# zzhang1987/Factor-Graph-Neural-Network

Measured on AMD Instinct MI355X. Metric: VF+FV messages/sec on 96.3.963 LDPC graph, higher is better.
Workload: dtype bf16

## Files before the change

factor-graph-neural-network_amd/csrc/bnact.hip:

```cpp
#include "fgnn_common.h"
#include "fgnn_device.h"
#include "fgnn_gridfold.h"
#include <stdlib.h>

#define BN_THREADS 256
#define BN_GRID 512
#define BN_MAXPART 1024
#define BN_APPLY_GRID 4096

struct BnParams {
    const void* x;
    const void* gy;
    void* out;
    float* ws;
    const float* a;
    const float* b;
    const float* gamma;
    const float* beta;
    const float* ref;
    const void* addend;
    const void* addend2;
    const void* addend3;
    int aperiod[3];
    int64_t R;
// ... 118 lines not shown
        for (int q = pg * 8; q < pg * 8 + 8; ++q) { a += red0[q * BN_FC + cc]; b += red1[q * BN_FC + cc]; }
    __syncthreads();
    if (pg < 8) { red0[threadIdx.x] = a; red1[threadIdx.x] = b; }
    __syncthreads();
    s0 = 0.0; s1 = 0.0;
    if (pg == 0)
        for (int q = 0; q < 8; ++q) { s0 += red0[q * BN_FC + cc]; s1 += red1[q * BN_FC + cc]; }
}

__global__ __launch_bounds__(256) void bn_stats_final_kernel(const float* ws, int nwg, int C, const fgnn_bn_final fin) {
    if (fin.num_batches_tracked && blockIdx.x == 0 && threadIdx.x == 0) *fin.num_batches_tracked += 1;
    const int c = blockIdx.x * BN_FC + (threadIdx.x & (BN_FC - 1)), pg = threadIdx.x / BN_FC;
    double s0, s1;
    bn_fold(ws, nwg, C, c, pg, c < C, s0, s1);
    if (pg != 0 || c >= C) return;
    const double n = (double)fin.count;
    const double m0 = s0 / n;
    double var = s1 / n - m0 * m0;
    if (var < 0.0) var = 0.0;
    const float mu = (float)(m0 + (fin.shift_k ? (double)fin.shift_k[c] : 0.0));
    const float is = (float)(1.0 / sqrt(var + (double)fin.eps));
    fin.mean[c] = mu;
    fin.invstd[c] = is;
    const float g = fin.gamma ? fin.gamma[c] : 1.f, b = fin.beta ? fin.beta[c] : 0.f;
    fin.scale[c] = g * is;
    fin.shift[c] = b - mu * g * is;
    if (fin.running_mean) {
        const double np = (double)(fin.population > 0 ? fin.population : fin.count);
        const double unbiased = np > 1.0 ? var * np / (np - 1.0) : var;
        fin.running_mean[c] = (1.f - fin.momentum) * fin.running_mean[c] + fin.momentum * mu;
        fin.running_var[c] = (1.f - fin.momentum) * fin.running_var[c] + fin.momentum * (float)unbiased;
    }
}

__global__ __launch_bounds__(256) void bn_bwd_final_kernel(const float* ws, int nwg, int C, float* dsum,
                                                           float* gweight, float* gbias) {
    const int c = blockIdx.x * BN_FC + (threadIdx.x & (BN_FC - 1)), pg = threadIdx.x / BN_FC;
    double s0, s1;
    bn_fold(ws, nwg, C, c, pg, c < C, s0, s1);
    if (pg != 0 || c >= C) return;
    dsum[c] = (float)s0;
    dsum[C + c] = (float)s1;
    if (gbias) gbias[c] += (float)s0;
    if (gweight) gweight[c] += (float)s1;
}

template <typename T, int MODE>
__global__ __launch_bounds__(BN_THREADS) void bn_apply_kernel(const BnParams p) {
    constexpr int EPC = Chunk<T>::EPC;
    const int tid = threadIdx.x;
    const int cpr = 1 << p.cshift;
    const int cg = tid & (cpr - 1), rg = tid >> p.cshift;
    const int rstep = BN_THREADS >> p.cshift;
    const int c0 = cg * EPC;
    const T* xg = static_cast<const T*>(p.x);
    const T* gg = static_cast<const T*>(p.gy);
    T* og = static_cast<T*>(p.out);
    float ka[EPC], kb[EPC], kc[EPC], kd[EPC], ke[EPC], kf[EPC];
#pragma unroll
// ... 77 lines not shown
}

extern "C" int64_t fgnn_bn_workspace_bytes(int64_t R, int C) { return (int64_t)BN_MAXPART * 2 * C * 4 + 2 * C * 4; }

static int g_inkernel_finalisers = -1;
int fgnn_separate_finalisers(void) {
    if (g_inkernel_finalisers < 0) g_inkernel_finalisers = 0;
    return !g_inkernel_finalisers;
}
extern "C" int fgnn_set_inkernel_finalisers(int on) {
    const int was = !fgnn_separate_finalisers();
    g_inkernel_finalisers = on ? 1 : 0;
    return was;
}

static int bn_check_final(const char* who, const fgnn_bn_final* fin) {
    if (!fin || !fin->mean || !fin->invstd || !fin->scale || !fin->shift) FGNN_FAIL(FGNN_EINVAL, "%s: null pointer in fgnn_bn_final", who);
    if (fin->count < 1 || (fin->population != 0 && fin->population < fin->count)) FGNN_FAIL(FGNN_EINVAL, "%s: bad row counts in fgnn_bn_final", who);
    if ((fin->running_mean == nullptr) != (fin->running_var == nullptr)) FGNN_FAIL(FGNN_EINVAL, "%s: running_mean and running_var go together", who);
    return FGNN_OK;
}

int fgnn_bn_finalize_launch(const float* partials, int npartials, int C, const fgnn_bn_final* fin, hipStream_t st) {
    hipLaunchKernelGGL(bn_stats_final_kernel, dim3((C + BN_FC - 1) / BN_FC), dim3(256), 0, st, partials, npartials, C, *fin);
    return hipGetLastError() == hipSuccess ? 0 : -1;
}

extern "C" int fgnn_bn_stats(const void* x, int64_t R, int C, int dtype, const fgnn_bn_final* fin, void* workspace,
                             int64_t workspace_bytes, void* fold_scratch, fgnn_stream_t stream) {
    BnParams p = {};
    int grid, rc;
    if (!x || !workspace) FGNN_FAIL(FGNN_EINVAL, "bn_stats: null pointer");
    if ((rc = bn_check_final("bn_stats", fin))) return rc;
    if (fin->count != R) FGNN_FAIL(FGNN_EINVAL, "bn_stats: fin->count must be R");
    if (bn_plan(R, C, dtype, &p, &grid)) FGNN_FAIL(FGNN_EUNSUPPORTED, "bn: C=%d not a supported channel count", C);
    if (workspace_bytes < fgnn_bn_workspace_bytes(R, C)) FGNN_FAIL(FGNN_EINVAL, "bn: workspace too small");
    float* ws = (float*)workspace;
    hipStream_t st = (hipStream_t)stream;
    const float* ref = dtype == FGNN_F32 ? (const float*)x : nullptr;
    p.x = x; p.ws = ws; p.ref = ref;
    p.fin = *fin;
    if (ref) {
        if (fin->shift_k) FGNN_FAIL(FGNN_EINVAL, "bn_stats: shift_k is for partials produced elsewhere");
        p.fin.shift_k = ref;
    }
    const bool inkernel = fold_scratch && 2 * C <= FGNN_FOLD_MAXJ && !fgnn_separate_finalisers();
    p.fold = fgnn_fold_make(ws, inkernel ? fold_scratch : nullptr, grid, C);
    if (dtype == FGNN_F32) hipLaunchKernelGGL((bn_reduce_kernel<float, 0>), dim3(grid), dim3(BN_THREADS), 0, st, p);
    else hipLaunchKernelGGL((bn_reduce_kernel<bf16_t, 0>), dim3(grid), dim3(BN_THREADS), 0, st, p);
    if (!inkernel) hipLaunchKernelGGL(bn_stats_final_kernel, dim3((C + BN_FC - 1) / BN_FC), dim3(256), 0, st, ws, grid, C, p.fin);
    hipError_t e = hipGetLastError();
    if (e != hipSuccess) FGNN_FAIL(FGNN_ELAUNCH, "bn_stats launch: %s", hipGetErrorString(e));
    return FGNN_OK;
}

extern "C" int fgnn_bn_finalize(const float* partials, int npartials, int C, const fgnn_bn_final* fin, fgnn_stream_t stream) {
    int rc;
    if (!partials) FGNN_FAIL(FGNN_EINVAL, "bn_finalize: null pointer");
    if ((rc = bn_check_final("bn_finalize", fin))) return rc;
    if (npartials < 1 || npartials > BN_MAXPART || C < 1) FGNN_FAIL(FGNN_EINVAL, "bn_finalize: bad sizes");
    if (fgnn_bn_finalize_launch(partials, npartials, C, fin, (hipStream_t)stream))
        FGNN_FAIL(FGNN_ELAUNCH, "bn_finalize launch: %s", hipGetErrorString(hipGetLastError()));
    return FGNN_OK;
}

extern "C" int fgnn_bn_apply(const void* x, void* y, int64_t R, int C, int dtype, const float* scale,
                             const float* shift, float slope, const void* addend, const void* addend2,
                             const void* addend3, const int32_t* addend_period, fgnn_stream_t stream) {
    BnParams p = {};
    int grid;
    if (!x || !y || !scale || !shift) FGNN_FAIL(FGNN_EINVAL, "bn_apply: null pointer");
    if (bn_plan(R, C, dtype, &p, &grid, bn_apply_grid())) FGNN_FAIL(FGNN_EUNSUPPORTED, "bn: C=%d not a supported channel count", C);
    p.x = x; p.out = y; p.a = scale; p.b = shift; p.slope = slope; p.addend = addend; p.addend2 = addend2; p.addend3 = addend3;
    for (int a = 0; a < 3; ++a) {
// ... 53 lines not shown
    pa.fold.tickets = nullptr;
    (void)bn_plan(R, C, dtype, &pa, &agrid, bn_apply_grid());
    if (dtype == FGNN_F32) hipLaunchKernelGGL((bn_apply_kernel<float, 1>), dim3(agrid), dim3(BN_THREADS), 0, st, pa);
    else hipLaunchKernelGGL((bn_apply_kernel<bf16_t, 1>), dim3(agrid), dim3(BN_THREADS), 0, st, pa);
    hipError_t e = hipGetLastError();
    if (e != hipSuccess) FGNN_FAIL(FGNN_ELAUNCH, "bn_backward launch: %s", hipGetErrorString(e));
    return FGNN_OK;
}

__global__ __launch_bounds__(256) void bn_bwd_final_raw_kernel(const float* ws, int nwg, int C, const float* mean,
                                                               const float* invstd, float* dsum, float* gweight, float* gbias) {
    const int c = blockIdx.x * BN_FC + (threadIdx.x & (BN_FC - 1)), pg = threadIdx.x / BN_FC;
    double s0, s1;
    bn_fold(ws, nwg, C, c, pg, c < C, s0, s1);
    if (pg != 0 || c >= C) return;
    const double dg = (double)invstd[c] * (s1 - (double)mean[c] * s0);
    dsum[c] = (float)s0;
    dsum[C + c] = (float)dg;
    if (gbias) gbias[c] += (float)s0;
    if (gweight) gweight[c] += (float)dg;
}

int fgnn_bn_bwd_final_raw_launch(const float* partials, int npartials, int C, const float* mean, const float* invstd, float* dsum,
                                 float* gweight, float* gbias, hipStream_t st) {
    hipLaunchKernelGGL(bn_bwd_final_raw_kernel, dim3((C + BN_FC - 1) / BN_FC), dim3(256), 0, st, partials, npartials, C, mean,
                       invstd, dsum, gweight, gbias);
    return hipGetLastError() == hipSuccess ? 0 : -1;
}

extern "C" int fgnn_bn_backward_apply(const void* x, const void* gy, void* gx, int64_t R, int C, int dtype,
                                      const float* mean, const float* invstd, const float* gamma, const float* beta,
                                      float slope, const float* dsum, fgnn_stream_t stream) {
    BnParams p = {};
    int grid;
    if (!x || !gy || !gx || !mean || !invstd || !gamma || !beta || !dsum)
// ... 12 lines not shown
```

factor-graph-neural-network_amd/csrc/fgnn_common.h:

```cpp
#pragma once
#include <hip/hip_runtime.h>
#include <stdint.h>
#include <stdio.h>
#include <stdarg.h>

#include "fgnn_hip.h"

typedef float f32x4 __attribute__((ext_vector_type(4)));

#define FGNN_THREADS 256
#define FGNN_WAVES 4

struct bf16_t { uint16_t v; };

__device__ __forceinline__ float fgnn_ld(const float* p) { return *p; }
__device__ __forceinline__ float fgnn_ld(const bf16_t* p) {
    return __uint_as_float(((uint32_t)p->v) << 16);
}
__device__ __forceinline__ void fgnn_st(float* p, float v) { *p = v; }
__device__ __forceinline__ void fgnn_st(bf16_t* p, float v) {
    const __bf16 h = (__bf16)v;
    p->v = __builtin_bit_cast(uint16_t, h);
}

// ... 18 lines not shown

#ifdef FGNN_ENABLE_PROF
long long* fgnn_prof_begin();
void fgnn_prof_print(const long long* prof, const char* tag, int first, int rows, int cols, int stride);
#else
static inline long long* fgnn_prof_begin() { return nullptr; }
static inline void fgnn_prof_print(const long long*, const char*, int, int, int, int) {}
#endif

static inline int fgnn_round_up(int v, int m) { return (v + m - 1) / m * m; }

void fgnn_launch_slab_reduce(const float* ws, int nslab, int64_t slab_len, int64_t nw, float* gW, float* gbias, hipStream_t st);
void fgnn_launch_slab_reduce_ld(const float* ws, int nslab, int64_t slab_len, int64_t nw, int ncols, int ld, float* gW,
                                float* gbias, hipStream_t st);
bool fgnn_fold_push(const float* ws, int nslab, int64_t slab_len, int64_t nw, float* gW, float* gb, int kind, int a, int b, int c, int d);
int fgnn_bn_finalize_launch(const float* partials, int npartials, int C, const fgnn_bn_final* fin, hipStream_t st);
int fgnn_bn_bwd_final_raw_launch(const float* partials, int npartials, int C, const float* mean, const float* invstd, float* dsum,
                                 float* gweight, float* gbias, hipStream_t st);
int fgnn_bn_backward_sums_bf16(const void* x, const void* gy, int64_t R, int C, const float* mean, const float* invstd,
                               const float* gamma, const float* beta, float slope, float* gweight, float* gbias,
                               void* workspace, void* fold_scratch, hipStream_t st, const float** dsum_out);
```

factor-graph-neural-network_amd/csrc/fgnn_gridfold.h:

```cpp
#pragma once
#include "fgnn_common.h"

#define FGNN_FOLD_GROUP 16
#define FGNN_FOLD_MAXGROUPS 64
#define FGNN_FOLD_MAXJ 512
#define FGNN_FOLD_TICKET_BYTES 512
#define FGNN_FOLD_BYTES (FGNN_FOLD_TICKET_BYTES + FGNN_FOLD_MAXGROUPS * FGNN_FOLD_MAXJ * 8)

struct FgnnFold {
    float* part;
    double* part2;
    unsigned* tickets;
    int rows;
    int row_stride, half_stride, ch;
};

static inline FgnnFold fgnn_fold_make(float* part, void* scratch, int rows, int ch, int row_stride = 0, int half_stride = 0) {
    FgnnFold f;
    f.part = part;
    f.tickets = (unsigned*)scratch;
    f.part2 = scratch ? (double*)((char*)scratch + FGNN_FOLD_TICKET_BYTES) : nullptr;
    f.rows = rows; f.ch = ch;
    f.row_stride = row_stride ? row_stride : 2 * ch;
    f.half_stride = half_stride ? half_stride : ch;
// ... 48 lines not shown
    if (!fgnn_fold_flag) return false;
    for (int j = tid; j < J; j += T) {
        double a = 0.0;
#pragma unroll 8
        for (int q = 0; q < ng; ++q) a += __hip_atomic_load(f.part2 + (int64_t)q * J + j, __ATOMIC_RELAXED, __HIP_MEMORY_SCOPE_AGENT);
        sums[j] = a;
    }
    if (tid == 0) __hip_atomic_store(f.tickets, 0u, __ATOMIC_RELAXED, __HIP_MEMORY_SCOPE_AGENT);
    __syncthreads();
    return true;
}


__device__ __forceinline__ void fgnn_bn_final_apply(const fgnn_bn_final& fin, int ch, const double* sums) {
    if (fin.num_batches_tracked && threadIdx.x == 0) *fin.num_batches_tracked += 1;
    for (int c = threadIdx.x; c < ch; c += blockDim.x) {
        const double n = (double)fin.count;
        const double m0 = sums[c] / n;
        double var = sums[ch + c] / n - m0 * m0;
        if (var < 0.0) var = 0.0;
        const float mu = (float)(m0 + (fin.shift_k ? (double)fin.shift_k[c] : 0.0));
        const float is = (float)(1.0 / sqrt(var + (double)fin.eps));
        fin.mean[c] = mu;
        fin.invstd[c] = is;
        const float g = fin.gamma ? fin.gamma[c] : 1.f, b = fin.beta ? fin.beta[c] : 0.f;
        fin.scale[c] = g * is;
        fin.shift[c] = b - mu * g * is;
        if (fin.running_mean) {
            const double np = (double)(fin.population > 0 ? fin.population : fin.count);
            const double unbiased = np > 1.0 ? var * np / (np - 1.0) : var;
            fin.running_mean[c] = (1.f - fin.momentum) * fin.running_mean[c] + fin.momentum * mu;
            fin.running_var[c] = (1.f - fin.momentum) * fin.running_var[c] + fin.momentum * (float)unbiased;
        }
    }
}

__device__ __forceinline__ void fgnn_bn_bwd_final_apply(int ch, const double* sums, const float* mean, const float* invstd,
                                                        float* dsum, float* gweight, float* gbias) {
    for (int c = threadIdx.x; c < ch; c += blockDim.x) {
        const double s0 = sums[c];
        const double s1 = mean ? (double)invstd[c] * (sums[ch + c] - (double)mean[c] * s0) : sums[ch + c];
        dsum[c] = (float)s0;
        dsum[ch + c] = (float)s1;
        if (gbias) gbias[c] += (float)s0;
        if (gweight) gweight[c] += (float)s1;
    }
}
#endif
```

factor-graph-neural-network_amd/fgnn_amd/_hip.py:

```python
import ctypes
import os
import re

import torch

_HERE = os.path.dirname(os.path.abspath(__file__))
LIB_PATH = os.environ.get('FGNN_HIP_LIB') or os.path.join(_HERE, 'libfgnn_hip.so')
HEADER_PATH = os.path.normpath(os.path.join(_HERE, '..', '..', 'include', 'fgnn_hip.h'))


class FgnnHipError(RuntimeError):
    pass


class MPConvDesc(ctypes.Structure):
    _fields_ = [(n, ctypes.c_int32) for n in
                ('B', 'nin', 'nou', 'net', 'N', 'M', 'k', 'ext', 'agg', 'dtype', 'relu', 'reserved')] + \
               [(n, ctypes.c_int64) for n in
                ('x_sb', 'x_sc', 'x_sn', 'idx_sb', 'idx_sm', 'idx_sk',
                 'et_sb', 'et_se', 'et_sm', 'et_sk', 'y_sb', 'y_sc', 'y_sm')]


class BnFinal(ctypes.Structure):
    _fields_ = [(n, ctypes.c_void_p) for n in ('gamma', 'beta', 'running_mean', 'running_var', 'num_batches_tracked',
# ... 77 lines not shown
            raise FgnnHipError('include/fgnn_hip.h: FGNN_%s = `%s` is not an integer expression' % (name, value.strip()))
        out[name] = int(eval(value, {'__builtins__': {}}))
    return out


def _header():
    if not os.path.exists(HEADER_PATH):
        raise FgnnHipError('the C-ABI header was not found at %s — the binding is derived from it and has no built-in '
                           'copy of the interface' % HEADER_PATH)
    with open(HEADER_PATH) as f:
        return f.read()


SIGNATURES, _K = (parse(_header()) for parse in (signatures, constants))
EXPORTS = tuple(SIGNATURES)
EXT_NONE, EXT_NEIGHBOR, EXT_DIFF = _K['EXT_NONE'], _K['EXT_NEIGHBOR'], _K['EXT_DIFF']
DESC_GETYPE_REDUCED = _K['DESC_GETYPE_REDUCED']
DESC_IDENTITY_LIST = _K['DESC_IDENTITY_LIST']
AGG_MAX, AGG_LSE, AGG_MEAN = _K['AGG_MAX'], _K['AGG_LSE'], _K['AGG_MEAN']
F32, BF16 = _K['F32'], _K['BF16']
DEC_F32, DEC_BF16, DEC_U8 = _K['DEC_F32'], _K['DEC_BF16'], _K['DEC_U8']
LABEL_I64, LABEL_U8 = _K['LABEL_I64'], _K['LABEL_U8']
PGM_DEC_F32, PGM_DEC_BF16, PGM_DEC_I64 = _K['PGM_DEC_F32'], _K['PGM_DEC_BF16'], _K['PGM_DEC_I64']
ABI_VERSION = _K['ABI_VERSION']
EUNSUPPORTED = _K['EUNSUPPORTED']
FOLD_SCRATCH_BYTES = _K['FOLD_SCRATCH_BYTES']

AGG_CODES = {'max': AGG_MAX, 'softmax': AGG_LSE, 'mean': AGG_MEAN}


# ... 91 lines not shown
```

factor-graph-neural-network_amd/fgnn_amd/mpnn/blocks.py:

```python
import ctypes

import torch

from .. import _hip, ops
from . import pointwise
from .message_op import _EXT_CODE, base_mp_nn, mp_conv_type, mp_conv_v2
from .pointwise import (BatchNormAct2d, BnHandoff, NodeInstanceNorm, PointwiseConv2d, _InstNormAct, _RowLinear, as_addends, node_sum,
                        refresh_in_place)
from .pointwise import state_epoch as pointwise_state_epoch


def _conv_norm_act(cin, cout, norm, act, bias=True):
    layers = [PointwiseConv2d(cin, cout, 1, bias=bias)]
    if norm is not None:
        layers.append(norm)
    layers.append(act)
    return torch.nn.Sequential(*layers)


FUSE_EVAL_BLOCKS = True


class iid_mapping(torch.nn.Module):
    def __init__(self, nin, nout, bias=True):
# ... 83 lines not shown
TAIL_WGRAD_MOMENTS = True
FUSE_TRAIN_TAIL = True


FUSE_TRAIN_HEAD = True


_HEAD_WIDTHS = (64, 128)


class _BlockHead(torch.autograd.Function):

    @staticmethod
    def forward(ctx, rows, weight, bias, bn_w, bn_b, handoff, slope, box=None):
        ctx.box = box
        z1 = pointwise.hip_linear(rows, weight, bias, bn=handoff)
        if z1 is None:
            raise _hip.FgnnHipError('fused block head: the 1x1 map is outside csrc/linear_fwd_b16.hip (checked by the caller)')
        R = rows.shape[0]
        stats = handoff.batch_stats(z1)
        a1 = torch.empty_like(z1)
        ops.timed('bn_apply (forward)', 2 * z1.numel() * 2, lambda: _hip.call(
            'fgnn_bn_apply', z1, a1, R, 64, _hip.BF16, stats[2], stats[3], slope, None, None, None, None))
        ctx.save_for_backward(rows, z1, stats, weight, bn_w, bn_b)
        ctx.slope = slope
        ctx.params = (weight, bias, bn_w, bn_b)
        return a1

    @staticmethod
    def backward(ctx, ga1):
        ops.backward_node_begins()
        L = _hip.lib()
        rows, z1, stats, weight, bn_w, bn_b = ctx.saved_tensors
        pW, pbias, pw, pb = ctx.params
        R, cin = rows.shape
        dev = rows.device
        ga1 = ga1.contiguous()
        if ga1.dtype != z1.dtype:
# ... 292 lines not shown
                return y
        M = ops.single_source_fanout(node_feature, nn_idx, etype) if (staged and not self.with_residual and addend is None
                                                                     and node_feature.shape[0] > 1) else 0
        if M:
            B, C = node_feature.shape[:2]
            one = node_feature.reshape(B, 1, 1, C).permute(0, 3, 1, 2)
            y1 = self._forward_staged(one, nn_idx[:, :1, :], etype[:, :, :1, :], None, M)
            return ops.broadcast_nodes(y1, M)
        return self._forward_staged(node_feature, nn_idx, etype, addend, 1)

    def _forward_staged(self, node_feature, nn_idx, etype, addend, mult):
        fuse = self.training
        h = self._fused_train_head(node_feature)
        if h is None:
            handoff = BnHandoff.of(self.conv1[1]) if fuse else None
            h = self.conv1[1](self.conv1[0](node_feature, bn=handoff), handoff=handoff)
        y = self._fused_train_tail(h, nn_idx, etype, addend, mult)
        if y is not None:
            return y + node_feature if self.with_residual else y
        h = self.mp_conv(h, nn_idx, etype, population_mult=mult)
        handoff = BnHandoff.of(self.conv2[1]) if (fuse and mult == 1) else None
        h = self.conv2[0](h, bn=handoff)
        if callable(addend):
            addend = addend()
        h = self.conv2[1](h, addend=addend, population_mult=mult, handoff=handoff)
        return h + node_feature if self.with_residual else h

    def _fused_train_head(self, x):
        conv, bn = self.conv1[0], self.conv1[1]
        handoff = BnHandoff.of(bn) if isinstance(bn, BatchNormAct2d) else None
        if not (FUSE_TRAIN_HEAD and self.training and torch.is_grad_enabled() and x.is_cuda and isinstance(conv, PointwiseConv2d)
# ... 75 lines not shown
```

factor-graph-neural-network_amd/fgnn_amd/mpnn/pointwise.py:

```python
import ctypes
import dataclasses
import weakref

import torch

from .. import _hip, ops


_CAST_CACHE = {}
_CAST_EPOCH = 0
_FLAT_MIRRORS = []


def invalidate_casts():
    global _CAST_EPOCH
    _CAST_EPOCH += 1


_STATE_EPOCH = 0


def note_state_change():
    global _STATE_EPOCH
    _STATE_EPOCH += 1
# ... 47 lines not shown
        v = _from_flat_mirror(t, dtype)
        if v is not None:
            return v
    key = id(t)
    hit = _CAST_CACHE.get(key)
    if hit is not None and hit[0]() is t and hit[3].dtype == dtype and hit[3].device == t.device and hit[3].shape == t.shape:
        if hit[1] != t._version or hit[2] != _CAST_EPOCH:
            hit[3].copy_(t.detach())
            hit[1], hit[2] = t._version, _CAST_EPOCH
        return hit[3]
    out = t.detach().to(dtype)
    _CAST_CACHE[key] = [weakref.ref(t, lambda _, key=key: _CAST_CACHE.pop(key, None)), t._version, _CAST_EPOCH, out]
    return out


@dataclasses.dataclass(eq=False)
class BnHandoff:
    gamma: torch.Tensor
    beta: torch.Tensor
    running_mean: torch.Tensor
    running_var: torch.Tensor
    num_batches_tracked: torch.Tensor
    momentum: float
    eps: float
    rows: torch.Tensor = dataclasses.field(default=None, init=False)
    stats: torch.Tensor = dataclasses.field(default=None, init=False)

    @classmethod
    def of(cls, bn):
        if bn is None or not bn.training or not bn.track_running_stats or not bn.affine or bn.momentum is None:
# ... 12 lines not shown
        note_state_change()
        self.rows, self.stats = rows, stats

    def stats_for(self, rows):
        if self.stats is not None and self.rows.data_ptr() == rows.data_ptr() and self.rows.shape == rows.shape:
            return self.stats
        return None

    def batch_stats(self, rows, population=0):
        stats = self.stats_for(rows)
        if stats is not None:
            return stats
        L = _hip.lib()
        R, C = rows.shape
        stats, fin = self.final(C, rows.device, R, population, running=self.stats is None)
        ws = ops._workspace(rows.device, int(L.fgnn_bn_workspace_bytes(R, C)))
        fold = ops._fold_scratch(rows.device)
        ops.timed('bn_stats (reduce + finalise)', rows.numel() * rows.element_size(), lambda: _hip.call(
            'fgnn_bn_stats', rows, R, C, _hip.dtype_code(rows), fin, ws, ws.numel() * 4, fold))
        note_state_change()
        return stats


def hip_linear(rows, weight, bias, bn=None, transposed=False):
    if not (rows.is_cuda and rows.dtype == torch.bfloat16 and weight.dtype == torch.float32 and rows.is_contiguous()):
        return None
    R, cin = rows.shape
    cout = weight.shape[1] if transposed else weight.shape[0]
    if cin * cout > (16384 if bn is not None else 8192):
        return None
# ... 251 lines not shown
            periods.append(1)
    return ts, periods


def period_array(periods):
    periods = (list(periods) + [1, 1, 1])[:3]
    return None if all(q == 1 for q in periods) else (ctypes.c_int32 * 3)(*periods)


class _BatchNormAct(torch.autograd.Function):

    @staticmethod
    def forward(ctx, rows, weight, bias, handoff, slope, addend=None, addend2=None, addend3=None, periods=(1, 1, 1), population=0):
        R, C = rows.shape
        dt = _hip.dtype_code(rows)
        stats = handoff.batch_stats(rows, population)
        y = torch.empty_like(rows)
        ctx.has_addend = tuple(a is not None for a in (addend, addend2, addend3))
        ctx.periods = tuple(periods)
        ops.timed('bn_apply (forward)', (2 + sum(ctx.has_addend)) * rows.numel() * rows.element_size(),
                  lambda: _hip.call('fgnn_bn_apply', rows, y, R, C, dt, stats[2], stats[3], slope, addend, addend2, addend3,
                                    period_array(periods)))
        ctx.save_for_backward(rows, weight, bias, stats)
        ctx.slope = slope
        ctx.params = (weight, bias)
        return y

    @staticmethod
    def backward(ctx, gy):
        ops.backward_node_begins()
        rows, weight, bias, stats = ctx.saved_tensors
        L = _hip.lib()
        R, C = rows.shape
        gy = gy.contiguous()
        if gy.dtype != rows.dtype:
            gy = gy.to(rows.dtype)
        gx = torch.empty_like(rows)
        grads = ops.param_grads(rows.device)
        gw, gb = grads.acc('gamma', ctx.params[0], (C,)), grads.acc('beta', ctx.params[1], (C,))
        ws = ops._workspace(rows.device, int(L.fgnn_bn_workspace_bytes(R, C)))
        fold = ops._fold_scratch(rows.device)
        ops.timed('bn_backward (reduce + finalise + apply)', 5 * rows.numel() * rows.element_size(),
                  lambda: _hip.call('fgnn_bn_backward', rows, gy, gx, R, C, _hip.dtype_code(rows), stats[0], stats[1], weight, bias,
                                    ctx.slope, gw, gb, ws, ws.numel() * 4, fold))
        ga = [None, None, None]
        for i in range(3):
            if ctx.has_addend[i] and ctx.needs_input_grad[5 + i]:
                ga[i] = gy if ctx.periods[i] == 1 else node_sum(gy, ctx.periods[i])
        return (gx, grads.result('gamma'), grads.result('beta'), None, None, *ga, None, None)


class BatchNormAct2d(torch.nn.BatchNorm2d):

    def __init__(self, num_features, slope=0.0):
        super().__init__(num_features)
        self.slope = float(slope)

    @staticmethod
    def _activate(y, slope):
# ... 59 lines not shown
```

Baseline: 2.001 billion.

## Add single-kernel few-rows BatchNorm stats+apply and backward paths

Adds a few-rows BatchNorm family where one workgroup owns 8 channels and loops over all rows. That lets stats, finalise and apply (or the backward reduce, finalise and apply) run in one kernel with no cross-block workspace fold or separate finaliser launch. The Python side routes small-R bf16 layers to it and skips the fused stats in the preceding linear. Shared finaliser formulas move into a header. The cost is low parallelism (C/8 blocks) and a second pass over the rows, which suits only small R.

```diff
diff --git a/factor-graph-neural-network_amd/csrc/bnact.hip b/factor-graph-neural-network_amd/csrc/bnact.hip
--- a/factor-graph-neural-network_amd/csrc/bnact.hip
+++ b/factor-graph-neural-network_amd/csrc/bnact.hip
@@ -156,23 +156,7 @@
     double s0, s1;
     bn_fold(ws, nwg, C, c, pg, c < C, s0, s1);
     if (pg != 0 || c >= C) return;
-    const double n = (double)fin.count;
-    const double m0 = s0 / n;
-    double var = s1 / n - m0 * m0;
-    if (var < 0.0) var = 0.0;
-    const float mu = (float)(m0 + (fin.shift_k ? (double)fin.shift_k[c] : 0.0));
-    const float is = (float)(1.0 / sqrt(var + (double)fin.eps));
-    fin.mean[c] = mu;
-    fin.invstd[c] = is;
-    const float g = fin.gamma ? fin.gamma[c] : 1.f, b = fin.beta ? fin.beta[c] : 0.f;
-    fin.scale[c] = g * is;
-    fin.shift[c] = b - mu * g * is;
-    if (fin.running_mean) {
-        const double np = (double)(fin.population > 0 ? fin.population : fin.count);
-        const double unbiased = np > 1.0 ? var * np / (np - 1.0) : var;
-        fin.running_mean[c] = (1.f - fin.momentum) * fin.running_mean[c] + fin.momentum * mu;
-        fin.running_var[c] = (1.f - fin.momentum) * fin.running_var[c] + fin.momentum * (float)unbiased;
-    }
+    fgnn_bn_final_channel(fin, c, s0, s1, fgnn_bn_final_shift(fin, c));
 }
 
 __global__ __launch_bounds__(256) void bn_bwd_final_kernel(const float* ws, int nwg, int C, float* dsum,
@@ -181,10 +165,7 @@
     double s0, s1;
     bn_fold(ws, nwg, C, c, pg, c < C, s0, s1);
     if (pg != 0 || c >= C) return;
-    dsum[c] = (float)s0;
-    dsum[C + c] = (float)s1;
-    if (gbias) gbias[c] += (float)s0;
-    if (gweight) gweight[c] += (float)s1;
+    fgnn_bn_bwd_final_channel(C, c, s0, s1, nullptr, nullptr, dsum, gweight, gbias);
 }
 
 template <typename T, int MODE>
@@ -292,7 +273,7 @@
     return was;
 }
 
-static int bn_check_final(const char* who, const fgnn_bn_final* fin) {
+int fgnn_bn_check_final(const char* who, const fgnn_bn_final* fin) {
     if (!fin || !fin->mean || !fin->invstd || !fin->scale || !fin->shift) FGNN_FAIL(FGNN_EINVAL, "%s: null pointer in fgnn_bn_final", who);
     if (fin->count < 1 || (fin->population != 0 && fin->population < fin->count)) FGNN_FAIL(FGNN_EINVAL, "%s: bad row counts in fgnn_bn_final", who);
     if ((fin->running_mean == nullptr) != (fin->running_var == nullptr)) FGNN_FAIL(FGNN_EINVAL, "%s: running_mean and running_var go together", who);
@@ -309,7 +290,7 @@
     BnParams p = {};
     int grid, rc;
     if (!x || !workspace) FGNN_FAIL(FGNN_EINVAL, "bn_stats: null pointer");
-    if ((rc = bn_check_final("bn_stats", fin))) return rc;
+    if ((rc = fgnn_bn_check_final("bn_stats", fin))) return rc;
     if (fin->count != R) FGNN_FAIL(FGNN_EINVAL, "bn_stats: fin->count must be R");
     if (bn_plan(R, C, dtype, &p, &grid)) FGNN_FAIL(FGNN_EUNSUPPORTED, "bn: C=%d not a supported channel count", C);
     if (workspace_bytes < fgnn_bn_workspace_bytes(R, C)) FGNN_FAIL(FGNN_EINVAL, "bn: workspace too small");
@@ -335,7 +316,7 @@
 extern "C" int fgnn_bn_finalize(const float* partials, int npartials, int C, const fgnn_bn_final* fin, fgnn_stream_t stream) {
     int rc;
     if (!partials) FGNN_FAIL(FGNN_EINVAL, "bn_finalize: null pointer");
-    if ((rc = bn_check_final("bn_finalize", fin))) return rc;
+    if ((rc = fgnn_bn_check_final("bn_finalize", fin))) return rc;
     if (npartials < 1 || npartials > BN_MAXPART || C < 1) FGNN_FAIL(FGNN_EINVAL, "bn_finalize: bad sizes");
     if (fgnn_bn_finalize_launch(partials, npartials, C, fin, (hipStream_t)stream))
         FGNN_FAIL(FGNN_ELAUNCH, "bn_finalize launch: %s", hipGetErrorString(hipGetLastError()));
@@ -419,11 +400,7 @@
     double s0, s1;
     bn_fold(ws, nwg, C, c, pg, c < C, s0, s1);
     if (pg != 0 || c >= C) return;
-    const double dg = (double)invstd[c] * (s1 - (double)mean[c] * s0);
-    dsum[c] = (float)s0;
-    dsum[C + c] = (float)dg;
-    if (gbias) gbias[c] += (float)s0;
-    if (gweight) gweight[c] += (float)dg;
+    fgnn_bn_bwd_final_channel(C, c, s0, s1, mean, invstd, dsum, gweight, gbias);
 }
 
 int fgnn_bn_bwd_final_raw_launch(const float* partials, int npartials, int C, const float* mean, const float* invstd, float* dsum,
diff --git a/factor-graph-neural-network_amd/csrc/few_rows.hip b/factor-graph-neural-network_amd/csrc/few_rows.hip
--- /dev/null
+++ b/factor-graph-neural-network_amd/csrc/few_rows.hip
@@ -0,0 +1,225 @@
+#include "fgnn_common.h"
+#include "fgnn_few_rows.h"
+#include "fgnn_device.h"
+#include "fgnn_bn_formulas.h"
+#include <stdlib.h>
+
+#define FR_THREADS 256
+#define FR_EPC 8
+#define FR_SLOTS (2 * FR_EPC)
+#define FR_PAD (FR_SLOTS + 1)
+
+struct FrParams {
+    const bf16_t* x;
+    const bf16_t* gy;
+    bf16_t* out;
+    const bf16_t* add[3];
+    int aperiod[3];
+    int R, C;
+    float slope;
+    fgnn_bn_final fin;
+    const float* mean;
+    const float* invstd;
+    const float* gamma;
+    const float* beta;
+    float* gweight;
+    float* gbias;
+};
+
+__device__ __forceinline__ void fr_load(const bf16_t* p, float (&v)[FR_EPC]) {
+    const uint4 t = *reinterpret_cast<const uint4*>(p);
+    v[0] = fgnn_lo(t.x); v[1] = fgnn_hi(t.x); v[2] = fgnn_lo(t.y); v[3] = fgnn_hi(t.y);
+    v[4] = fgnn_lo(t.z); v[5] = fgnn_hi(t.z); v[6] = fgnn_lo(t.w); v[7] = fgnn_hi(t.w);
+}
+__device__ __forceinline__ void fr_store(bf16_t* p, const float (&v)[FR_EPC]) {
+    *reinterpret_cast<uint4*>(p) = make_uint4(fgnn_pack2(v[0], v[1]), fgnn_pack2(v[2], v[3]), fgnn_pack2(v[4], v[5]), fgnn_pack2(v[6], v[7]));
+}
+
+__device__ __forceinline__ void fr_fold(const float (&s0)[FR_EPC], const float (&s1)[FR_EPC], float* part, double* lvl1, double* tot) {
+    const int tid = threadIdx.x;
+#pragma unroll
+    for (int e = 0; e < FR_EPC; ++e) { part[tid * FR_PAD + e] = s0[e]; part[tid * FR_PAD + FR_EPC + e] = s1[e]; }
+    __syncthreads();
+    const int slot = tid & (FR_SLOTS - 1), grp = tid / FR_SLOTS;
+    double a = 0.0;
+#pragma unroll
+    for (int q = 0; q < 16; ++q) a += (double)part[(grp * 16 + q) * FR_PAD + slot];
+    lvl1[grp * FR_SLOTS + slot] = a;
+    __syncthreads();
+    if (tid < FR_SLOTS) {
+        a = 0.0;
+#pragma unroll
+        for (int q = 0; q < FR_THREADS / 16; ++q) a += lvl1[q * FR_SLOTS + tid];
+        tot[tid] = a;
+    }
+    __syncthreads();
+}
+
+__global__ __launch_bounds__(FR_THREADS) void bn_rows_fwd_kernel(const FrParams p) {
+    __shared__ float part[FR_THREADS * FR_PAD];
+    __shared__ double lvl1[(FR_THREADS / 16) * FR_SLOTS], tot[FR_SLOTS];
+    __shared__ float kss[FR_SLOTS];
+    const int tid = threadIdx.x;
+    const int c0 = blockIdx.x * FR_EPC;
+    float k[FR_EPC], s0[FR_EPC], s1[FR_EPC];
+    fr_load(p.x + c0, k);
+#pragma unroll
+    for (int e = 0; e < FR_EPC; ++e) { s0[e] = 0.f; s1[e] = 0.f; }
+#pragma unroll 4
+    for (int r = tid; r < p.R; r += FR_THREADS) {
+        float v[FR_EPC];
+        fr_load(p.x + r * p.C + c0, v);
+#pragma unroll
+        for (int e = 0; e < FR_EPC; ++e) { const float dlt = v[e] - k[e]; s0[e] += dlt; s1[e] = fmaf(dlt, dlt, s1[e]); }
+    }
+    fr_fold(s0, s1, part, lvl1, tot);
+    if (p.fin.num_batches_tracked && blockIdx.x == 0 && tid == 0) *p.fin.num_batches_tracked += 1;
+    if (tid < FR_EPC) {
+        fgnn_bn_final_channel(p.fin, c0 + tid, tot[tid], tot[FR_EPC + tid], (double)k[tid]);
+        kss[tid] = p.fin.scale[c0 + tid];
+        kss[FR_EPC + tid] = p.fin.shift[c0 + tid];
+    }
+    if (!p.out) return;
+    __syncthreads();
+    float sc[FR_EPC], sh[FR_EPC];
+#pragma unroll
+    for (int e = 0; e < FR_EPC; ++e) { sc[e] = kss[e]; sh[e] = kss[FR_EPC + e]; }
+#pragma unroll 4
+    for (int r = tid; r < p.R; r += FR_THREADS) {
+        float v[FR_EPC], o[FR_EPC];
+        fr_load(p.x + r * p.C + c0, v);
+#pragma unroll
+        for (int e = 0; e < FR_EPC; ++e) o[e] = fgnn_bn_act(v[e], sc[e], sh[e], p.slope);
+#pragma unroll
+        for (int a = 0; a < 3; ++a) {
+            if (p.add[a]) {
+                float ad[FR_EPC];
+                const int ar = p.aperiod[a] > 1 ? r / p.aperiod[a] : r;
+                fr_load(p.add[a] + ar * p.C + c0, ad);
+#pragma unroll
+                for (int e = 0; e < FR_EPC; ++e) o[e] += ad[e];
+            }
+        }
+        fr_store(p.out + r * p.C + c0, o);
+    }
+}
+
+__global__ __launch_bounds__(FR_THREADS) void bn_rows_bwd_kernel(const FrParams p) {
+    __shared__ float part[FR_THREADS * FR_PAD];
+    __shared__ double lvl1[(FR_THREADS / 16) * FR_SLOTS], tot[FR_SLOTS];
+    __shared__ float dsum[FR_SLOTS];
+    const int tid = threadIdx.x;
+    const int c0 = blockIdx.x * FR_EPC;
+    float mu[FR_EPC], is[FR_EPC], sc[FR_EPC], sh[FR_EPC], s0[FR_EPC], s1[FR_EPC];
+#pragma unroll
+    for (int e = 0; e < FR_EPC; ++e) {
+        mu[e] = p.mean[c0 + e];
+        is[e] = p.invstd[c0 + e];
+        sc[e] = p.gamma[c0 + e] * is[e];
+        sh[e] = p.beta[c0 + e] - mu[e] * sc[e];
+        s0[e] = 0.f; s1[e] = 0.f;
+    }
+#pragma unroll 4
+    for (int r = tid; r < p.R; r += FR_THREADS) {
+        float v[FR_EPC], g[FR_EPC];
+        fr_load(p.x + r * p.C + c0, v);
+        fr_load(p.gy + r * p.C + c0, g);
+#pragma unroll
+        for (int e = 0; e < FR_EPC; ++e) {
+            const float ge = fgnn_bn_act_grad(v[e], g[e], sc[e], sh[e], p.slope);
+            s0[e] += ge;
+            s1[e] = fmaf(ge, (v[e] - mu[e]) * is[e], s1[e]);
+        }
+    }
+    fr_fold(s0, s1, part, lvl1, tot);
+    if (tid < FR_EPC)
+        fgnn_bn_bwd_final_channel(FR_EPC, tid, tot[tid], tot[FR_EPC + tid], nullptr, nullptr, dsum, p.gweight ? p.gweight + c0 : nullptr,
+                                  p.gbias ? p.gbias + c0 : nullptr);
+    __syncthreads();
+    const float inv_r = 1.0f / (float)p.R;
+    float db[FR_EPC], dg[FR_EPC];
+#pragma unroll
+    for (int e = 0; e < FR_EPC; ++e) { db[e] = dsum[e] * inv_r; dg[e] = dsum[FR_EPC + e] * inv_r; }
+#pragma unroll 4
+    for (int r = tid; r < p.R; r += FR_THREADS) {
+        float v[FR_EPC], g[FR_EPC], o[FR_EPC];
+        fr_load(p.x + r * p.C + c0, v);
+        fr_load(p.gy + r * p.C + c0, g);
+#pragma unroll
+        for (int e = 0; e < FR_EPC; ++e) {
+            const float ge = fgnn_bn_act_grad(v[e], g[e], sc[e], sh[e], p.slope);
+            const float xh = (v[e] - mu[e]) * is[e];
+            o[e] = sc[e] * (ge - db[e] - xh * dg[e]);
+        }
+        fr_store(p.out + r * p.C + c0, o);
+    }
+}
+
+static int g_few_rows = -1;
+static int few_rows_on(void) {
+    if (g_few_rows < 0) {
+        const char* e = getenv("FGNN_FEW_ROWS");
+        g_few_rows = (e && e[0] == '0') ? 0 : 1;
+    }
+    return g_few_rows;
+}
+extern "C" int fgnn_set_few_rows(int32_t on) {
+    const int was = few_rows_on();
+    g_few_rows = on ? 1 : 0;
+    return was;
+}
+
+static int fr_plan(int64_t R, int C, int dtype, int* grid) {
+    if (dtype != FGNN_BF16) return 0;
+    if (R < 1 || R > FGNN_FEW_ROWS_MAX) return 0;
+    if (C < FR_EPC || C > FGNN_FEW_ROWS_MAX_C || C % FR_EPC != 0) return 0;
+    *grid = C / FR_EPC;
+    return 1;
+}
+static bool fr_aligned(const void* p) { return ((uintptr_t)p & 15) == 0; }
+
+extern "C" int fgnn_bn_rows_supported(int64_t R, int32_t C, int32_t dtype) {
+    int grid;
+    return few_rows_on() && fr_plan(R, C, dtype, &grid);
+}
+
+extern "C" int fgnn_bn_rows_forward(const void* x, void* y, int64_t R, int32_t C, int32_t dtype, const fgnn_bn_final* fin, float slope,
+                                    const void* addend, const void* addend2, const void* addend3, const int32_t* addend_period,
+                                    fgnn_stream_t stream) {
+    FrParams p = {};
+    int grid, rc;
+    if (!x) FGNN_FAIL(FGNN_EINVAL, "bn_rows_forward: null pointer");
+    if (!fr_plan(R, C, dtype, &grid)) FGNN_FAIL(FGNN_EUNSUPPORTED, "bn_rows_forward: R=%lld C=%d dtype=%d is outside the few-rows family", (long long)R, C, dtype);
+    if ((rc = fgnn_bn_check_final("bn_rows_forward", fin))) return rc;
+    if (fin->count != R) FGNN_FAIL(FGNN_EINVAL, "bn_rows_forward: fin->count must be R");
+    if (fin->shift_k) FGNN_FAIL(FGNN_EINVAL, "bn_rows_forward: shift_k is for partials produced elsewhere");
+    const void* ads[3] = {addend, addend2, addend3};
+    if (!fr_aligned(x) || !fr_aligned(y) || !fr_aligned(addend) || !fr_aligned(addend2) || !fr_aligned(addend3))
+        FGNN_FAIL(FGNN_EUNSUPPORTED, "bn_rows_forward: tensors must be 16-byte aligned");
+    for (int a = 0; a < 3; ++a) {
+        p.add[a] = (const bf16_t*)ads[a];
+        p.aperiod[a] = addend_period ? addend_period[a] : 1;
+        if (p.aperiod[a] < 1) FGNN_FAIL(FGNN_EINVAL, "bn_rows_forward: addend period < 1");
+    }
+    p.x = (const bf16_t*)x; p.out = (bf16_t*)y; p.R = (int)R; p.C = C; p.slope = slope; p.fin = *fin;
+    hipLaunchKernelGGL(bn_rows_fwd_kernel, dim3(grid), dim3(FR_THREADS), 0, (hipStream_t)stream, p);
+    hipError_t e = hipGetLastError();
+    if (e != hipSuccess) FGNN_FAIL(FGNN_ELAUNCH, "bn_rows_forward launch: %s", hipGetErrorString(e));
+    return FGNN_OK;
+}
+
+extern "C" int fgnn_bn_rows_backward(const void* x, const void* gy, void* gx, int64_t R, int32_t C, int32_t dtype, const float* mean,
+                                     const float* invstd, const float* gamma, const float* beta, float slope, float* gweight,
+                                     float* gbias, fgnn_stream_t stream) {
+    FrParams p = {};
+    int grid;
+    if (!x || !gy || !gx || !mean || !invstd || !gamma || !beta) FGNN_FAIL(FGNN_EINVAL, "bn_rows_backward: null pointer");
+    if (!fr_plan(R, C, dtype, &grid)) FGNN_FAIL(FGNN_EUNSUPPORTED, "bn_rows_backward: R=%lld C=%d dtype=%d is outside the few-rows family", (long long)R, C, dtype);
+    if (!fr_aligned(x) || !fr_aligned(gy) || !fr_aligned(gx)) FGNN_FAIL(FGNN_EUNSUPPORTED, "bn_rows_backward: tensors must be 16-byte aligned");
+    p.x = (const bf16_t*)x; p.gy = (const bf16_t*)gy; p.out = (bf16_t*)gx; p.R = (int)R; p.C = C; p.slope = slope;
+    p.mean = mean; p.invstd = invstd; p.gamma = gamma; p.beta = beta; p.gweight = gweight; p.gbias = gbias;
+    hipLaunchKernelGGL(bn_rows_bwd_kernel, dim3(grid), dim3(FR_THREADS), 0, (hipStream_t)stream, p);
+    hipError_t e = hipGetLastError();
+    if (e != hipSuccess) FGNN_FAIL(FGNN_ELAUNCH, "bn_rows_backward launch: %s", hipGetErrorString(e));
+    return FGNN_OK;
+}
diff --git a/factor-graph-neural-network_amd/csrc/fgnn_bn_formulas.h b/factor-graph-neural-network_amd/csrc/fgnn_bn_formulas.h
--- /dev/null
+++ b/factor-graph-neural-network_amd/csrc/fgnn_bn_formulas.h
@@ -0,0 +1,47 @@
+#pragma once
+#include "fgnn_common.h"
+
+#ifdef __HIPCC__
+__device__ __forceinline__ void fgnn_bn_final_channel(const fgnn_bn_final& fin, int c, double s0, double s1, double k) {
+    const double n = (double)fin.count;
+    const double m0 = s0 / n;
+    double var = s1 / n - m0 * m0;
+    if (var < 0.0) var = 0.0;
+    const float mu = (float)(m0 + k);
+    const float is = (float)(1.0 / sqrt(var + (double)fin.eps));
+    fin.mean[c] = mu;
+    fin.invstd[c] = is;
+    const float g = fin.gamma ? fin.gamma[c] : 1.f, b = fin.beta ? fin.beta[c] : 0.f;
+    fin.scale[c] = g * is;
+    fin.shift[c] = b - mu * g * is;
+    if (fin.running_mean) {
+        const double np = (double)(fin.population > 0 ? fin.population : fin.count);
+        const double unbiased = np > 1.0 ? var * np / (np - 1.0) : var;
+        fin.running_mean[c] = (1.f - fin.momentum) * fin.running_mean[c] + fin.momentum * mu;
+        fin.running_var[c] = (1.f - fin.momentum) * fin.running_var[c] + fin.momentum * (float)unbiased;
+    }
+}
+
+__device__ __forceinline__ double fgnn_bn_final_shift(const fgnn_bn_final& fin, int c) {
+    return fin.shift_k ? (double)fin.shift_k[c] : 0.0;
+}
+
+__device__ __forceinline__ void fgnn_bn_bwd_final_channel(int ch, int c, double s0, double s1, const float* mean, const float* invstd,
+                                                          float* dsum, float* gweight, float* gbias) {
+    const double dg = mean ? (double)invstd[c] * (s1 - (double)mean[c] * s0) : s1;
+    if (dsum) {
+        dsum[c] = (float)s0;
+        dsum[ch + c] = (float)dg;
+    }
+    if (gbias) gbias[c] += (float)s0;
+    if (gweight) gweight[c] += (float)dg;
+}
+
+__device__ __forceinline__ float fgnn_bn_act(float x, float scale, float shift, float slope) {
+    const float pre = fmaf(x, scale, shift);
+    return pre > 0.f ? pre : pre * slope;
+}
+__device__ __forceinline__ float fgnn_bn_act_grad(float x, float gy, float scale, float shift, float slope) {
+    return fmaf(x, scale, shift) > 0.f ? gy : gy * slope;
+}
+#endif
diff --git a/factor-graph-neural-network_amd/csrc/fgnn_common.h b/factor-graph-neural-network_amd/csrc/fgnn_common.h
--- a/factor-graph-neural-network_amd/csrc/fgnn_common.h
+++ b/factor-graph-neural-network_amd/csrc/fgnn_common.h
@@ -56,6 +56,7 @@
 void fgnn_launch_slab_reduce_ld(const float* ws, int nslab, int64_t slab_len, int64_t nw, int ncols, int ld, float* gW,
                                 float* gbias, hipStream_t st);
 bool fgnn_fold_push(const float* ws, int nslab, int64_t slab_len, int64_t nw, float* gW, float* gb, int kind, int a, int b, int c, int d);
+int fgnn_bn_check_final(const char* who, const fgnn_bn_final* fin);
 int fgnn_bn_finalize_launch(const float* partials, int npartials, int C, const fgnn_bn_final* fin, hipStream_t st);
 int fgnn_bn_bwd_final_raw_launch(const float* partials, int npartials, int C, const float* mean, const float* invstd, float* dsum,
                                  float* gweight, float* gbias, hipStream_t st);
diff --git a/factor-graph-neural-network_amd/csrc/fgnn_gridfold.h b/factor-graph-neural-network_amd/csrc/fgnn_gridfold.h
--- a/factor-graph-neural-network_amd/csrc/fgnn_gridfold.h
+++ b/factor-graph-neural-network_amd/csrc/fgnn_gridfold.h
@@ -1,5 +1,6 @@
 #pragma once
 #include "fgnn_common.h"
+#include "fgnn_bn_formulas.h"
 
 #define FGNN_FOLD_GROUP 16
 #define FGNN_FOLD_MAXGROUPS 64
@@ -86,36 +87,11 @@
 
 __device__ __forceinline__ void fgnn_bn_final_apply(const fgnn_bn_final& fin, int ch, const double* sums) {
     if (fin.num_batches_tracked && threadIdx.x == 0) *fin.num_batches_tracked += 1;
-    for (int c = threadIdx.x; c < ch; c += blockDim.x) {
-        const double n = (double)fin.count;
-        const double m0 = sums[c] / n;
-        double var = sums[ch + c] / n - m0 * m0;
-        if (var < 0.0) var = 0.0;
-        const float mu = (float)(m0 + (fin.shift_k ? (double)fin.shift_k[c] : 0.0));
-        const float is = (float)(1.0 / sqrt(var + (double)fin.eps));
-        fin.mean[c] = mu;
-        fin.invstd[c] = is;
-        const float g = fin.gamma ? fin.gamma[c] : 1.f, b = fin.beta ? fin.beta[c] : 0.f;
-        fin.scale[c] = g * is;
-        fin.shift[c] = b - mu * g * is;
-        if (fin.running_mean) {
-            const double np = (double)(fin.population > 0 ? fin.population : fin.count);
-            const double unbiased = np > 1.0 ? var * np / (np - 1.0) : var;
-            fin.running_mean[c] = (1.f - fin.momentum) * fin.running_mean[c] + fin.momentum * mu;
-            fin.running_var[c] = (1.f - fin.momentum) * fin.running_var[c] + fin.momentum * (float)unbiased;
-        }
-    }
+    for (int c = threadIdx.x; c < ch; c += blockDim.x) fgnn_bn_final_channel(fin, c, sums[c], sums[ch + c], fgnn_bn_final_shift(fin, c));
 }
 
 __device__ __forceinline__ void fgnn_bn_bwd_final_apply(int ch, const double* sums, const float* mean, const float* invstd,
                                                         float* dsum, float* gweight, float* gbias) {
-    for (int c = threadIdx.x; c < ch; c += blockDim.x) {
-        const double s0 = sums[c];
-        const double s1 = mean ? (double)invstd[c] * (sums[ch + c] - (double)mean[c] * s0) : sums[ch + c];
-        dsum[c] = (float)s0;
-        dsum[ch + c] = (float)s1;
-        if (gbias) gbias[c] += (float)s0;
-        if (gweight) gweight[c] += (float)s1;
-    }
+    for (int c = threadIdx.x; c < ch; c += blockDim.x) fgnn_bn_bwd_final_channel(ch, c, sums[c], sums[ch + c], mean, invstd, dsum, gweight, gbias);
 }
 #endif
diff --git a/factor-graph-neural-network_amd/fgnn_amd/_hip.py b/factor-graph-neural-network_amd/fgnn_amd/_hip.py
--- a/factor-graph-neural-network_amd/fgnn_amd/_hip.py
+++ b/factor-graph-neural-network_amd/fgnn_amd/_hip.py
@@ -7,6 +7,7 @@
 _HERE = os.path.dirname(os.path.abspath(__file__))
 LIB_PATH = os.environ.get('FGNN_HIP_LIB') or os.path.join(_HERE, 'libfgnn_hip.so')
 HEADER_PATH = os.path.normpath(os.path.join(_HERE, '..', '..', 'include', 'fgnn_hip.h'))
+ANNEX_PATHS = (os.path.normpath(os.path.join(_HERE, '..', '..', 'include', 'fgnn_few_rows.h')),)
 
 
 class FgnnHipError(RuntimeError):
@@ -115,6 +116,15 @@
 
 SIGNATURES, _K = (parse(_header()) for parse in (signatures, constants))
 EXPORTS = tuple(SIGNATURES)
+ANNEX_CONSTANTS = {}
+for _path in ANNEX_PATHS:
+    with open(_path) as _f:
+        _text = _f.read()
+    _clash = set(signatures(_text)) & set(SIGNATURES)
+    if _clash:
+        raise FgnnHipError('%s declares %s a second time' % (_path, sorted(_clash)))
+    SIGNATURES.update(signatures(_text))
+    ANNEX_CONSTANTS.update(constants(_text))
 EXT_NONE, EXT_NEIGHBOR, EXT_DIFF = _K['EXT_NONE'], _K['EXT_NEIGHBOR'], _K['EXT_DIFF']
 DESC_GETYPE_REDUCED = _K['DESC_GETYPE_REDUCED']
 DESC_IDENTITY_LIST = _K['DESC_IDENTITY_LIST']
diff --git a/factor-graph-neural-network_amd/fgnn_amd/mpnn/blocks.py b/factor-graph-neural-network_amd/fgnn_amd/mpnn/blocks.py
--- a/factor-graph-neural-network_amd/fgnn_amd/mpnn/blocks.py
+++ b/factor-graph-neural-network_amd/fgnn_amd/mpnn/blocks.py
@@ -121,14 +121,21 @@
     @staticmethod
     def forward(ctx, rows, weight, bias, bn_w, bn_b, handoff, slope, box=None):
         ctx.box = box
-        z1 = pointwise.hip_linear(rows, weight, bias, bn=handoff)
+        few = bool(_hip.lib().fgnn_bn_rows_supported(rows.shape[0], 64, _hip.BF16)) and rows.shape[1] * 64 <= 8192
+        z1 = pointwise.hip_linear(rows, weight, bias, bn=None if few else handoff)
         if z1 is None:
             raise _hip.FgnnHipError('fused block head: the 1x1 map is outside csrc/linear_fwd_b16.hip (checked by the caller)')
         R = rows.shape[0]
-        stats = handoff.batch_stats(z1)
         a1 = torch.empty_like(z1)
-        ops.timed('bn_apply (forward)', 2 * z1.numel() * 2, lambda: _hip.call(
-            'fgnn_bn_apply', z1, a1, R, 64, _hip.BF16, stats[2], stats[3], slope, None, None, None, None))
+        if handoff.stats_for(z1) is None and pointwise.few_rows(z1):
+            stats, fin = handoff.final(64, z1.device, R)
+            ops.timed('bn_stats + apply (few rows: bn_rows_fwd_kernel)', 2 * z1.numel() * 2, lambda: _hip.call(
+                'fgnn_bn_rows_forward', z1, a1, R, 64, _hip.BF16, fin, slope, None, None, None, None))
+            pointwise.note_state_change()
+        else:
+            stats = handoff.batch_stats(z1)
+            ops.timed('bn_apply (forward)', 2 * z1.numel() * 2, lambda: _hip.call(
+                'fgnn_bn_apply', z1, a1, R, 64, _hip.BF16, stats[2], stats[3], slope, None, None, None, None))
         ctx.save_for_backward(rows, z1, stats, weight, bn_w, bn_b)
         ctx.slope = slope
         ctx.params = (weight, bias, bn_w, bn_b)
@@ -451,7 +458,8 @@
         h = self._fused_train_head(node_feature)
         if h is None:
             handoff = BnHandoff.of(self.conv1[1]) if fuse else None
-            h = self.conv1[1](self.conv1[0](node_feature, bn=handoff), handoff=handoff)
+            lean = handoff is not None and pointwise.few_rows_behind_map(node_feature, self.conv1[0].out_channels)
+            h = self.conv1[1](self.conv1[0](node_feature, bn=None if lean else handoff), handoff=handoff)
         y = self._fused_train_tail(h, nn_idx, etype, addend, mult)
         if y is not None:
             return y + node_feature if self.with_residual else y
diff --git a/factor-graph-neural-network_amd/fgnn_amd/mpnn/pointwise.py b/factor-graph-neural-network_amd/fgnn_amd/mpnn/pointwise.py
--- a/factor-graph-neural-network_amd/fgnn_amd/mpnn/pointwise.py
+++ b/factor-graph-neural-network_amd/fgnn_amd/mpnn/pointwise.py
@@ -85,6 +85,20 @@
     return out
 
 
+def few_rows(rows, *others):
+    if not (rows.is_cuda and rows.dtype == torch.bfloat16 and rows.dim() == 2 and rows.is_contiguous()):
+        return False
+    if any(t is not None and (t.dtype != rows.dtype or t.data_ptr() % 16) for t in (rows,) + others):
+        return False
+    return bool(_hip.lib().fgnn_bn_rows_supported(rows.shape[0], rows.shape[1], _hip.BF16))
+
+
+def few_rows_behind_map(x, cout):
+    dt = torch.get_autocast_dtype('cuda') if torch.is_autocast_enabled() else x.dtype
+    return bool(x.is_cuda and dt == torch.bfloat16 and x.shape[1] * cout <= 8192 and
+                _hip.lib().fgnn_bn_rows_supported(x.shape[0] * x.shape[2] * x.shape[3], cout, _hip.BF16))
+
+
 @dataclasses.dataclass(eq=False)
 class BnHandoff:
     gamma: torch.Tensor
@@ -127,6 +141,11 @@
         L = _hip.lib()
         R, C = rows.shape
         stats, fin = self.final(C, rows.device, R, population, running=self.stats is None)
+        if few_rows(rows):
+            ops.timed('bn_stats (few rows: bn_rows_fwd_kernel)', rows.numel() * rows.element_size(), lambda: _hip.call(
+                'fgnn_bn_rows_forward', rows, None, R, C, _hip.BF16, fin, 1.0, None, None, None, None))
+            note_state_change()
+            return stats
         ws = ops._workspace(rows.device, int(L.fgnn_bn_workspace_bytes(R, C)))
         fold = ops._fold_scratch(rows.device)
         ops.timed('bn_stats (reduce + finalise)', rows.numel() * rows.element_size(), lambda: _hip.call(
@@ -408,13 +427,20 @@
     def forward(ctx, rows, weight, bias, handoff, slope, addend=None, addend2=None, addend3=None, periods=(1, 1, 1), population=0):
         R, C = rows.shape
         dt = _hip.dtype_code(rows)
-        stats = handoff.batch_stats(rows, population)
         y = torch.empty_like(rows)
         ctx.has_addend = tuple(a is not None for a in (addend, addend2, addend3))
         ctx.periods = tuple(periods)
-        ops.timed('bn_apply (forward)', (2 + sum(ctx.has_addend)) * rows.numel() * rows.element_size(),
-                  lambda: _hip.call('fgnn_bn_apply', rows, y, R, C, dt, stats[2], stats[3], slope, addend, addend2, addend3,
-                                    period_array(periods)))
+        nbytes = (2 + sum(ctx.has_addend)) * rows.numel() * rows.element_size()
+        if handoff.stats_for(rows) is None and few_rows(rows, addend, addend2, addend3):
+            stats, fin = handoff.final(C, rows.device, R, population, running=handoff.stats is None)
+            ops.timed('bn_stats + apply (few rows: bn_rows_fwd_kernel)', nbytes, lambda: _hip.call(
+                'fgnn_bn_rows_forward', rows, y, R, C, dt, fin, slope, addend, addend2, addend3, period_array(periods)))
+            note_state_change()
+        else:
+            stats = handoff.batch_stats(rows, population)
+            ops.timed('bn_apply (forward)', nbytes,
+                      lambda: _hip.call('fgnn_bn_apply', rows, y, R, C, dt, stats[2], stats[3], slope, addend, addend2, addend3,
+                                        period_array(periods)))
         ctx.save_for_backward(rows, weight, bias, stats)
         ctx.slope = slope
         ctx.params = (weight, bias)
@@ -432,11 +458,16 @@
         gx = torch.empty_like(rows)
         grads = ops.param_grads(rows.device)
         gw, gb = grads.acc('gamma', ctx.params[0], (C,)), grads.acc('beta', ctx.params[1], (C,))
-        ws = ops._workspace(rows.device, int(L.fgnn_bn_workspace_bytes(R, C)))
-        fold = ops._fold_scratch(rows.device)
-        ops.timed('bn_backward (reduce + finalise + apply)', 5 * rows.numel() * rows.element_size(),
-                  lambda: _hip.call('fgnn_bn_backward', rows, gy, gx, R, C, _hip.dtype_code(rows), stats[0], stats[1], weight, bias,
-                                    ctx.slope, gw, gb, ws, ws.numel() * 4, fold))
+        if few_rows(rows, gy):
+            ops.timed('bn_backward (few rows: bn_rows_bwd_kernel)', 5 * rows.numel() * rows.element_size(),
+                      lambda: _hip.call('fgnn_bn_rows_backward', rows, gy, gx, R, C, _hip.BF16, stats[0], stats[1], weight, bias,
+                                        ctx.slope, gw, gb))
+        else:
+            ws = ops._workspace(rows.device, int(L.fgnn_bn_workspace_bytes(R, C)))
+            fold = ops._fold_scratch(rows.device)
+            ops.timed('bn_backward (reduce + finalise + apply)', 5 * rows.numel() * rows.element_size(),
+                      lambda: _hip.call('fgnn_bn_backward', rows, gy, gx, R, C, _hip.dtype_code(rows), stats[0], stats[1], weight, bias,
+                                        ctx.slope, gw, gb, ws, ws.numel() * 4, fold))
         ga = [None, None, None]
         for i in range(3):
             if ctx.has_addend[i] and ctx.needs_input_grad[5 + i]:
diff --git a/include/fgnn_few_rows.h b/include/fgnn_few_rows.h
--- /dev/null
+++ b/include/fgnn_few_rows.h
@@ -0,0 +1,23 @@
+#ifndef FGNN_FEW_ROWS_H
+#define FGNN_FEW_ROWS_H
+#include "fgnn_hip.h"
+
+#ifdef __cplusplus
+extern "C" {
+#endif
+
+#define FGNN_FEW_ROWS_MAX 8192
+#define FGNN_FEW_ROWS_MAX_C 1024
+int fgnn_set_few_rows(int32_t on);
+int fgnn_bn_rows_supported(int64_t R, int32_t C, int32_t dtype);
+int fgnn_bn_rows_forward(const void* x, void* y, int64_t R, int32_t C, int32_t dtype, const fgnn_bn_final* fin, float slope,
+                         const void* addend, const void* addend2, const void* addend3, const int32_t* addend_period,
+                         fgnn_stream_t stream);
+int fgnn_bn_rows_backward(const void* x, const void* gy, void* gx, int64_t R, int32_t C, int32_t dtype, const float* mean,
+                          const float* invstd, const float* gamma, const float* beta, float slope, float* gweight, float* gbias,
+                          fgnn_stream_t stream);
+
+#ifdef __cplusplus
+}
+#endif
+#endif
```

Measured after the change: 1.980 billion. 1.1% lower.
